# BatsResearch/menghini-neurips23-code

Measured on AMD Instinct MI355X. Metric: images/sec CLIP ViT-B/16 encode+prompt-step, higher is better.
Workload: dtype f16

## Files before the change

menghini-neurips23-code_amd/csrc/attention_split.hip:

```cpp
#include <math.h>

#include "common.h"

__device__ __forceinline__ int vt_index_fwd_s(int key, int d) { return vt_index(key, ((d >> 2) & 3) * 16 + (d >> 4) * 4 + (d & 3)); }

__device__ __forceinline__ void split8(const f32x4 a, const f32x4 b, half8& hi, half8& lo) {
    half4 h0, l0, h1, l1;
    split_f16x4(a, h0, l0);
    split_f16x4(b, h1, l1);
    hi = (half8){h0[0], h0[1], h0[2], h0[3], h1[0], h1[1], h1[2], h1[3]};
    lo = (half8){l0[0], l0[1], l0[2], l0[3], l1[0], l1[1], l1[2], l1[3]};
}

template <int KVC, bool CAUSAL, int NW>
__global__ __launch_bounds__(NW * 64) void attn_fwd_split_kernel(const float* __restrict__ qkv, half_t* __restrict__ out, int S, int H) {
    constexpr int SP = KVC * 32;
    constexpr float LOG2E = 1.4426950408889634f;
    constexpr float INV = 1.0f / (float)GRIP_SPLIT_LO_SCALE;
    extern __shared__ __attribute__((aligned(16))) char smem[];
    half_t* Kh = (half_t*)smem;
    half_t* Kl = Kh + SP * 64;
    half_t* Vh = Kl + SP * 64;
    half_t* Vl = Vh + SP * 64;

    const int tid = threadIdx.x, lane = tid & 63, wave = tid >> 6;
    const int D = H * 64;
    const int b = blockIdx.x / H, h = blockIdx.x - b * H;
    const size_t ld = (size_t)3 * D;
    const float* base = qkv + (size_t)b * S * ld + h * 64;
    const int li = lane & 15, lg = lane >> 4;
    const int n_qt = (S + 15) >> 4;

    for (int idx = tid; idx < SP * 8; idx += NW * 64) {
        const int row = idx >> 3, chunk = idx & 7;
        f32x4 a = {0.f, 0.f, 0.f, 0.f}, c = {0.f, 0.f, 0.f, 0.f};
        if (row < S) {
            const f32x4* p = (const f32x4*)(base + (size_t)row * ld + D + chunk * 8);
            a = p[0];
            c = p[1];
        }
        half8 hi, lo;
        split8(a, c, hi, lo);
        const int o = row * 64 + ((chunk ^ (row & 7)) * 8);
        *(half8*)(Kh + o) = hi;
        *(half8*)(Kl + o) = lo;
    }
    for (int idx = tid; idx < ((SP / 2 + 31) / 32) * 256; idx += NW * 64) {
        const int lane_rp = idx & 31, chunk = ((idx >> 5) & 1) + 2 * ((idx >> 6) & 3), rblk = idx >> 8;
        const int r0 = 2 * (rblk * 32 + lane_rp);
        if (r0 >= SP) continue;
        f32x4 z = {0.f, 0.f, 0.f, 0.f};
        f32x4 a0 = z, a1 = z, b0 = z, b1 = z;
        if (r0 < S) { const f32x4* p = (const f32x4*)(base + (size_t)r0 * ld + 2 * D + chunk * 8); a0 = p[0]; a1 = p[1]; }
        if (r0 + 1 < S) { const f32x4* p = (const f32x4*)(base + (size_t)(r0 + 1) * ld + 2 * D + chunk * 8); b0 = p[0]; b1 = p[1]; }
        half8 h0, l0, h1, l1;
        split8(a0, a1, h0, l0);
        split8(b0, b1, h1, l1);
#pragma unroll
        for (int j = 0; j < 8; ++j) {
            const int o = vt_index_fwd_s(r0, chunk * 8 + j);
            *(half2v*)(Vh + o) = (half2v){h0[j], h1[j]};
            *(half2v*)(Vl + o) = (half2v){l0[j], l1[j]};
        }
    }
    __syncthreads();

    for (int qt = wave; qt < n_qt; qt += NW) {
        asm volatile("" ::: "memory");
        const int qrow = qt * 16 + li;
        const int qr = qrow < S ? qrow : S - 1;
        half8 qh[2], ql[2];
#pragma unroll
        for (int kk = 0; kk < 2; ++kk) {
            const f32x4* p = (const f32x4*)(base + (size_t)qr * ld + (kk * 4 + lg) * 8);
            split8(p[0] * 0.125f, p[1] * 0.125f, qh[kk], ql[kk]);
        }
        f32x4 sc[2 * KVC];
        float m = -INFINITY;
#pragma unroll
        for (int t = 0; t < 2 * KVC; ++t) {
            f32x4 acc = {0.f, 0.f, 0.f, 0.f}, cor = {0.f, 0.f, 0.f, 0.f};
#pragma unroll
            for (int kk = 0; kk < 2; ++kk) {
                const int o = (t * 16 + li) * 64 + (((kk * 4 + lg) ^ (lane & 7)) * 8);
                const half8 kh = *(const half8*)(Kh + o), kl = *(const half8*)(Kl + o);
                acc = __builtin_amdgcn_mfma_f32_16x16x32_f16(kh, qh[kk], acc, 0, 0, 0);
                cor = __builtin_amdgcn_mfma_f32_16x16x32_f16(kl, qh[kk], cor, 0, 0, 0);
                cor = __builtin_amdgcn_mfma_f32_16x16x32_f16(kh, ql[kk], cor, 0, 0, 0);
            }
            acc += cor * INV;
            if (CAUSAL || t >= 2 * (KVC - 1)) {
#pragma unroll
                for (int r = 0; r < 4; ++r) {
                    const int kv = t * 16 + lg * 4 + r;
                    if (kv >= S || (CAUSAL && kv > qrow)) acc[r] = -INFINITY;
                }
            }
            m = fmaxf(fmaxf(fmaxf(m, acc[0]), fmaxf(acc[1], acc[2])), acc[3]);
            sc[t] = acc;
        }
        m = fmaxf(m, __shfl_xor(m, 16));
        m = fmaxf(m, __shfl_xor(m, 32));
        const float m2 = m * LOG2E;
#pragma unroll
        for (int t = 0; t < 2 * KVC; ++t)
#pragma unroll
            for (int r = 0; r < 4; ++r) sc[t][r] = __builtin_amdgcn_exp2f(__builtin_fmaf(sc[t][r], LOG2E, -m2));

        const half8 ones = {1, 1, 1, 1, 1, 1, 1, 1};
        f32x4 sum_h = {0.f, 0.f, 0.f, 0.f}, sum_l = {0.f, 0.f, 0.f, 0.f};
        f32x4 o[4], oc[4];
#pragma unroll
        for (int nf = 0; nf < 4; ++nf) { o[nf] = (f32x4){0.f, 0.f, 0.f, 0.f}; oc[nf] = (f32x4){0.f, 0.f, 0.f, 0.f}; }
#pragma unroll
        for (int c = 0; c < KVC; ++c) {
            half8 ph, pl;
            split8(sc[2 * c], sc[2 * c + 1], ph, pl);
#pragma unroll
            for (int nf = 0; nf < 4; ++nf) {
                const int vo = (c * 4 + nf) * 512 + (lg * 16 + (li ^ lg)) * 8;
                const half8 vh = *(const half8*)(Vh + vo), vl = *(const half8*)(Vl + vo);
                o[nf] = __builtin_amdgcn_mfma_f32_16x16x32_f16(vh, ph, o[nf], 0, 0, 0);
                oc[nf] = __builtin_amdgcn_mfma_f32_16x16x32_f16(vl, ph, oc[nf], 0, 0, 0);
                oc[nf] = __builtin_amdgcn_mfma_f32_16x16x32_f16(vh, pl, oc[nf], 0, 0, 0);
            }
            sum_h = __builtin_amdgcn_mfma_f32_16x16x32_f16(ones, ph, sum_h, 0, 0, 0);
            sum_l = __builtin_amdgcn_mfma_f32_16x16x32_f16(ones, pl, sum_l, 0, 0, 0);
        }
        if (qrow < S) {
            const float inv = 1.0f / (sum_h[0] + sum_l[0] * INV);
            half_t* orow = out + (size_t)((size_t)b * S + qrow) * 2 * D;
            const int col = h * 64 + lg * 16;
            half_t* op = orow + (col >> 5) * 64 + (col & 31);
            half8 hi0, lo0, hi1, lo1;
            split8((o[0] + oc[0] * INV) * inv, (o[1] + oc[1] * INV) * inv, hi0, lo0);
            split8((o[2] + oc[2] * INV) * inv, (o[3] + oc[3] * INV) * inv, hi1, lo1);
            *(half8*)op = hi0;
            *(half8*)(op + 8) = hi1;
            *(half8*)(op + 32) = lo0;
            *(half8*)(op + 40) = lo1;
        }
    }
}

bool attention_split_supported(int S) { return S >= 1 && S <= 320; }

int launch_attention_fwd_split(const float* qkv, void* out, int B, int S, int H, int causal, hipStream_t s) {
    GRIP_REQUIRE(attention_split_supported(S) && B >= 1 && H >= 1, "attention_split: bad shape B=%d S=%d H=%d (S <= 320)", B, S, H);
    const int kvc = (S + 31) / 32;
    const size_t lds = (size_t)4 * kvc * 32 * 64 * sizeof(half_t);
#define GRIP_ATT_CASE(K)                                                                                                                     \
    case K: {                                                                                                                                \
        static bool configured = false;                                                                                                      \
        if (!configured) {                                                                                                                   \
            GRIP_CHECK_HIP(hipFuncSetAttribute((const void*)attn_fwd_split_kernel<K, false, (K >= 4 ? 8 : 4)>, hipFuncAttributeMaxDynamicSharedMemorySize, (int)lds)); \
            GRIP_CHECK_HIP(hipFuncSetAttribute((const void*)attn_fwd_split_kernel<K, true, (K >= 4 ? 8 : 4)>, hipFuncAttributeMaxDynamicSharedMemorySize, (int)lds));  \
            configured = true;                                                                                                               \
        }                                                                                                                                    \
        if (causal) hipLaunchKernelGGL((attn_fwd_split_kernel<K, true, (K >= 4 ? 8 : 4)>), dim3(B * H), dim3((K >= 4 ? 8 : 4) * 64), lds, s, qkv, (half_t*)out, S, H); \
        else hipLaunchKernelGGL((attn_fwd_split_kernel<K, false, (K >= 4 ? 8 : 4)>), dim3(B * H), dim3((K >= 4 ? 8 : 4) * 64), lds, s, qkv, (half_t*)out, S, H);       \
    } break;
    switch (kvc) {
        GRIP_ATT_CASE(1) GRIP_ATT_CASE(2) GRIP_ATT_CASE(3) GRIP_ATT_CASE(4) GRIP_ATT_CASE(5)
        GRIP_ATT_CASE(6) GRIP_ATT_CASE(7) GRIP_ATT_CASE(8) GRIP_ATT_CASE(9) GRIP_ATT_CASE(10)
        default: GRIP_REQUIRE(false, "attention_split: S = %d out of range", S);
    }
#undef GRIP_ATT_CASE
    GRIP_CHECK_HIP(hipGetLastError());
    return GRIP_OK;
}
```

Before: 20760.

## Add persistent split-attention kernel overlapping next head's K/V loads with compute

```diff
diff --git a/menghini-neurips23-code_amd/csrc/attention_split.hip b/menghini-neurips23-code_amd/csrc/attention_split.hip
--- a/menghini-neurips23-code_amd/csrc/attention_split.hip
+++ b/menghini-neurips23-code_amd/csrc/attention_split.hip
@@ -12,11 +12,95 @@
     lo = (half8){l0[0], l0[1], l0[2], l0[3], l1[0], l1[1], l1[2], l1[3]};
 }
 
+template <int KVC, bool CAUSAL, class Store>
+__device__ __forceinline__ void attn_split_tile(const half_t* Kh, const half_t* Kl, const half_t* Vh, const half_t* Vl, const half8 (&qh)[2], const half8 (&ql)[2],
+                                                int qrow, int S, int lane, Store&& store) {
+    constexpr float LOG2E = 1.4426950408889634f;
+    constexpr float INV = 1.0f / (float)GRIP_SPLIT_LO_SCALE;
+    const int li = lane & 15, lg = lane >> 4;
+    f32x4 sc[2 * KVC];
+    float m = -INFINITY;
+    half8 kh[2][2], kl[2][2];
+    auto read_k = [&](int t) {
+#pragma unroll
+        for (int kk = 0; kk < 2; ++kk) {
+            const int o = (t * 16 + li) * 64 + (((kk * 4 + lg) ^ (lane & 7)) * 8);
+            kh[t & 1][kk] = *(const half8*)(Kh + o);
+            kl[t & 1][kk] = *(const half8*)(Kl + o);
+        }
+    };
+    read_k(0);
+#pragma unroll
+    for (int t = 0; t < 2 * KVC; ++t) {
+        if (t + 1 < 2 * KVC) read_k(t + 1);
+        f32x4 acc = {0.f, 0.f, 0.f, 0.f}, cor = {0.f, 0.f, 0.f, 0.f};
+#pragma unroll
+        for (int kk = 0; kk < 2; ++kk) {
+            acc = __builtin_amdgcn_mfma_f32_16x16x32_f16(kh[t & 1][kk], qh[kk], acc, 0, 0, 0);
+            cor = __builtin_amdgcn_mfma_f32_16x16x32_f16(kl[t & 1][kk], qh[kk], cor, 0, 0, 0);
+            cor = __builtin_amdgcn_mfma_f32_16x16x32_f16(kh[t & 1][kk], ql[kk], cor, 0, 0, 0);
+        }
+        acc += cor * INV;
+        if (CAUSAL || t >= 2 * (KVC - 1)) {
+#pragma unroll
+            for (int r = 0; r < 4; ++r) {
+                const int kv = t * 16 + lg * 4 + r;
+                if (kv >= S || (CAUSAL && kv > qrow)) acc[r] = -INFINITY;
+            }
+        }
+        m = fmaxf(fmaxf(fmaxf(m, acc[0]), fmaxf(acc[1], acc[2])), acc[3]);
+        sc[t] = acc;
+    }
+    m = fmaxf(m, __shfl_xor(m, 16));
+    m = fmaxf(m, __shfl_xor(m, 32));
+    const float m2 = m * LOG2E;
+#pragma unroll
+    for (int t = 0; t < 2 * KVC; ++t)
+#pragma unroll
+        for (int r = 0; r < 4; ++r) sc[t][r] = __builtin_amdgcn_exp2f(__builtin_fmaf(sc[t][r], LOG2E, -m2));
+
+    const half8 ones = {1, 1, 1, 1, 1, 1, 1, 1};
+    f32x4 sum_h = {0.f, 0.f, 0.f, 0.f}, sum_l = {0.f, 0.f, 0.f, 0.f};
+    f32x4 o[4], oc[4];
+#pragma unroll
+    for (int nf = 0; nf < 4; ++nf) { o[nf] = (f32x4){0.f, 0.f, 0.f, 0.f}; oc[nf] = (f32x4){0.f, 0.f, 0.f, 0.f}; }
+    half8 vh[2], vl[2];
+    auto read_v = [&](int st) {
+        const int vo = st * 512 + (lg * 16 + (li ^ lg)) * 8;
+        vh[st & 1] = *(const half8*)(Vh + vo);
+        vl[st & 1] = *(const half8*)(Vl + vo);
+    };
+    read_v(0);
+#pragma unroll
+    for (int c = 0; c < KVC; ++c) {
+        half8 ph, pl;
+        split8(sc[2 * c], sc[2 * c + 1], ph, pl);
+#pragma unroll
+        for (int nf = 0; nf < 4; ++nf) {
+            const int st = c * 4 + nf;
+            if (st + 1 < 4 * KVC) read_v(st + 1);
+            o[nf] = __builtin_amdgcn_mfma_f32_16x16x32_f16(vh[st & 1], ph, o[nf], 0, 0, 0);
+            oc[nf] = __builtin_amdgcn_mfma_f32_16x16x32_f16(vl[st & 1], ph, oc[nf], 0, 0, 0);
+            oc[nf] = __builtin_amdgcn_mfma_f32_16x16x32_f16(vh[st & 1], pl, oc[nf], 0, 0, 0);
+        }
+        sum_h = __builtin_amdgcn_mfma_f32_16x16x32_f16(ones, ph, sum_h, 0, 0, 0);
+        sum_l = __builtin_amdgcn_mfma_f32_16x16x32_f16(ones, pl, sum_l, 0, 0, 0);
+    }
+    const float inv = 1.0f / (sum_h[0] + sum_l[0] * INV);
+    half8 hi0, lo0, hi1, lo1;
+    split8((o[0] + oc[0] * INV) * inv, (o[1] + oc[1] * INV) * inv, hi0, lo0);
+    split8((o[2] + oc[2] * INV) * inv, (o[3] + oc[3] * INV) * inv, hi1, lo1);
+    store(hi0, hi1, lo0, lo1);
+}
+
+__device__ __forceinline__ int split_out_col(int h, int lane) {
+    const int col = h * 64 + (lane >> 4) * 16;
+    return (col >> 5) * 64 + (col & 31);
+}
+
 template <int KVC, bool CAUSAL, int NW>
 __global__ __launch_bounds__(NW * 64) void attn_fwd_split_kernel(const float* __restrict__ qkv, half_t* __restrict__ out, int S, int H) {
     constexpr int SP = KVC * 32;
-    constexpr float LOG2E = 1.4426950408889634f;
-    constexpr float INV = 1.0f / (float)GRIP_SPLIT_LO_SCALE;
     extern __shared__ __attribute__((aligned(16))) char smem[];
     half_t* Kh = (half_t*)smem;
     half_t* Kl = Kh + SP * 64;
@@ -65,6 +149,7 @@
     }
     __syncthreads();
 
+    half_t* orow = out + (size_t)b * S * 2 * D + split_out_col(h, lane);
     for (int qt = wave; qt < n_qt; qt += NW) {
         asm volatile("" ::: "memory");
         const int qrow = qt * 16 + li;
@@ -75,79 +160,225 @@
             const f32x4* p = (const f32x4*)(base + (size_t)qr * ld + (kk * 4 + lg) * 8);
             split8(p[0] * 0.125f, p[1] * 0.125f, qh[kk], ql[kk]);
         }
-        f32x4 sc[2 * KVC];
-        float m = -INFINITY;
-#pragma unroll
-        for (int t = 0; t < 2 * KVC; ++t) {
-            f32x4 acc = {0.f, 0.f, 0.f, 0.f}, cor = {0.f, 0.f, 0.f, 0.f};
-#pragma unroll
-            for (int kk = 0; kk < 2; ++kk) {
-                const int o = (t * 16 + li) * 64 + (((kk * 4 + lg) ^ (lane & 7)) * 8);
-                const half8 kh = *(const half8*)(Kh + o), kl = *(const half8*)(Kl + o);
-                acc = __builtin_amdgcn_mfma_f32_16x16x32_f16(kh, qh[kk], acc, 0, 0, 0);
-                cor = __builtin_amdgcn_mfma_f32_16x16x32_f16(kl, qh[kk], cor, 0, 0, 0);
-                cor = __builtin_amdgcn_mfma_f32_16x16x32_f16(kh, ql[kk], cor, 0, 0, 0);
+        attn_split_tile<KVC, CAUSAL>(Kh, Kl, Vh, Vl, qh, ql, qrow, S, lane, [&](half8 hi0, half8 hi1, half8 lo0, half8 lo1) {
+            if (qrow < S) {
+                half_t* op = orow + (size_t)qrow * 2 * D;
+                *(half8*)op = hi0;
+                *(half8*)(op + 8) = hi1;
+                *(half8*)(op + 32) = lo0;
+                *(half8*)(op + 40) = lo1;
             }
-            acc += cor * INV;
-            if (CAUSAL || t >= 2 * (KVC - 1)) {
-#pragma unroll
-                for (int r = 0; r < 4; ++r) {
-                    const int kv = t * 16 + lg * 4 + r;
-                    if (kv >= S || (CAUSAL && kv > qrow)) acc[r] = -INFINITY;
+        });
+    }
+}
+
+template <int KVC>
+__global__ __launch_bounds__(512) void attn_fwd_split_persistent_kernel(const float* __restrict__ qkv, half_t* __restrict__ out, int S, int H, int n_items) {
+    constexpr int NW = 8;
+    constexpr int SP = KVC * 32;
+    constexpr int NK = SP * 16 / (NW * 64);
+    constexpr int V_UNITS = ((SP / 2 + 31) / 32) * 256;
+    constexpr int NV = (V_UNITS + NW * 64 - 1) / (NW * 64);
+    static_assert(2 * KVC > NW && 2 * KVC <= 2 * NW, "one or two query tiles per wave");
+    extern __shared__ __attribute__((aligned(16))) char smem[];
+    half_t* Kh = (half_t*)smem;
+    half_t* Kl = Kh + SP * 64;
+    half_t* Vh = Kl + SP * 64;
+    half_t* Vl = Vh + SP * 64;
+
+    const int tid = threadIdx.x;
+    const int wave = __builtin_amdgcn_readfirstlane(tid >> 6);
+    const int D = H * 64;
+    const size_t ld = (size_t)3 * D;
+    const int n_qt = (S + 15) >> 4;
+
+    f32x4 kr[NK], vr[NV][4];
+    f32x4 qr[2][2];
+    half8 qh[2], ql[2];
+    const unsigned ldb = (unsigned)ld * 4;
+    const unsigned odb = (unsigned)D * 4;
+    auto fresh_tid = [&]() {
+        int t = tid;
+        asm volatile("" : "+v"(t));
+        return t;
+    };
+    auto in_rsrc = [&](int item) {
+        const int b = __builtin_amdgcn_readfirstlane(item / H), h = item - b * H;
+        return __builtin_amdgcn_make_buffer_rsrc((void*)(qkv + (size_t)b * S * ld + h * 64), 0, (int)((unsigned)(S - 1) * ldb + (unsigned)(2 * D + 64) * 4), 0x00020000);
+    };
+    auto out_rsrc = [&](int item) {
+        const int b = __builtin_amdgcn_readfirstlane(item / H);
+        return __builtin_amdgcn_make_buffer_rsrc((void*)(out + (size_t)b * S * 2 * D), 0, (int)((unsigned)S * odb), 0x00020000);
+    };
+    auto ldg = [&](__amdgpu_buffer_rsrc_t rs, unsigned off) { return __builtin_bit_cast(f32x4, __builtin_amdgcn_raw_buffer_load_b128(rs, (int)off, 0, 0)); };
+    auto load_k = [&](__amdgpu_buffer_rsrc_t rs) {
+        const int t = fresh_tid();
+        const unsigned ko = (unsigned)(t >> 4) * ldb + (unsigned)(D + (t & 15) * 4) * 4;
+#pragma unroll
+        for (int n = 0; n < NK; ++n) kr[n] = ldg(rs, ko + n * 32 * ldb);
+    };
+    auto load_v = [&](__amdgpu_buffer_rsrc_t rs) {
+        const int t = fresh_tid();
+        const int v_r0 = 2 * ((t >> 8) * 32 + (t & 31)), v_chunk = ((t >> 5) & 1) + 2 * ((t >> 6) & 3);
+        const unsigned vo = (unsigned)v_r0 * ldb + (unsigned)(2 * D + v_chunk * 8) * 4;
+#pragma unroll
+        for (int n = 0; n < NV; ++n) {
+            vr[n][0] = ldg(rs, vo + n * 128 * ldb);
+            vr[n][1] = ldg(rs, vo + n * 128 * ldb + 16);
+            vr[n][2] = ldg(rs, vo + (n * 128 + 1) * ldb);
+            vr[n][3] = ldg(rs, vo + (n * 128 + 1) * ldb + 16);
+        }
+    };
+    auto load_q = [&](__amdgpu_buffer_rsrc_t rs, int qt) {
+        const int t = fresh_tid();
+        const int qrow = qt * 16 + (t & 15);
+        const unsigned q_off = (unsigned)(qrow < S ? qrow : S - 1) * ldb + (unsigned)((t >> 4) & 3) * 32;
+#pragma unroll
+        for (int kk = 0; kk < 2; ++kk) {
+            qr[kk][0] = ldg(rs, q_off + kk * 128);
+            qr[kk][1] = ldg(rs, q_off + kk * 128 + 16);
+        }
+    };
+    auto split_q = [&]() {
+#pragma unroll
+        for (int kk = 0; kk < 2; ++kk) split8(qr[kk][0] * 0.125f, qr[kk][1] * 0.125f, qh[kk], ql[kk]);
+    };
+    auto stage_kv = [&]() {
+        const int t = fresh_tid();
+        const int k_r0 = t >> 4, k_q = t & 15;
+        half_t* kp = Kh + k_r0 * 64 + (((k_q >> 1) ^ (k_r0 & 7)) * 8) + (k_q & 1) * 4;
+#pragma unroll
+        for (int n = 0; n < NK; ++n) {
+            half4 hi, lo;
+            split_f16x4(kr[n], hi, lo);
+            *(half4*)(kp + n * 2048) = hi;
+            *(half4*)(kp + n * 2048 + SP * 64) = lo;
+        }
+        const int v_r0 = 2 * ((t >> 8) * 32 + (t & 31)), v_chunk = ((t >> 5) & 1) + 2 * ((t >> 6) & 3);
+        const int v_lg = (v_r0 >> 2) & 3;
+        const int v_lds = vt_index_fwd_s(v_r0, v_chunk * 8) ^ (v_lg * 8);
+        int v_st[4];
+#pragma unroll
+        for (int jj = 0; jj < 4; ++jj) {
+            v_st[jj] = 2 * SP * 64 + v_lds + ((jj ^ v_lg) * 8);
+            asm volatile("" : "+v"(v_st[jj]));
+        }
+        half8 vh[NV][2], vl[NV][2];
+#pragma unroll
+        for (int n = 0; n < NV; ++n) {
+            split8(vr[n][0], vr[n][1], vh[n][0], vl[n][0]);
+            split8(vr[n][2], vr[n][3], vh[n][1], vl[n][1]);
+        }
+#pragma unroll
+        for (int n = 0; n < NV; ++n) {
+            if (v_r0 + n * 128 < SP) {
+#pragma unroll
+                for (int j = 0; j < 8; ++j) {
+                    half_t* o = Kh + v_st[j & 3] + (n * 8192 + (j >> 2) * 512);
+                    *(half2v*)o = (half2v){vh[n][0][j], vh[n][1][j]};
+                    *(half2v*)(o + SP * 64) = (half2v){vl[n][0][j], vl[n][1][j]};
                 }
             }
-            m = fmaxf(fmaxf(fmaxf(m, acc[0]), fmaxf(acc[1], acc[2])), acc[3]);
-            sc[t] = acc;
-        }
-        m = fmaxf(m, __shfl_xor(m, 16));
-        m = fmaxf(m, __shfl_xor(m, 32));
-        const float m2 = m * LOG2E;
-#pragma unroll
-        for (int t = 0; t < 2 * KVC; ++t)
-#pragma unroll
-            for (int r = 0; r < 4; ++r) sc[t][r] = __builtin_amdgcn_exp2f(__builtin_fmaf(sc[t][r], LOG2E, -m2));
-
-        const half8 ones = {1, 1, 1, 1, 1, 1, 1, 1};
-        f32x4 sum_h = {0.f, 0.f, 0.f, 0.f}, sum_l = {0.f, 0.f, 0.f, 0.f};
-        f32x4 o[4], oc[4];
-#pragma unroll
-        for (int nf = 0; nf < 4; ++nf) { o[nf] = (f32x4){0.f, 0.f, 0.f, 0.f}; oc[nf] = (f32x4){0.f, 0.f, 0.f, 0.f}; }
-#pragma unroll
-        for (int c = 0; c < KVC; ++c) {
-            half8 ph, pl;
-            split8(sc[2 * c], sc[2 * c + 1], ph, pl);
-#pragma unroll
-            for (int nf = 0; nf < 4; ++nf) {
-                const int vo = (c * 4 + nf) * 512 + (lg * 16 + (li ^ lg)) * 8;
-                const half8 vh = *(const half8*)(Vh + vo), vl = *(const half8*)(Vl + vo);
-                o[nf] = __builtin_amdgcn_mfma_f32_16x16x32_f16(vh, ph, o[nf], 0, 0, 0);
-                oc[nf] = __builtin_amdgcn_mfma_f32_16x16x32_f16(vl, ph, oc[nf], 0, 0, 0);
-                oc[nf] = __builtin_amdgcn_mfma_f32_16x16x32_f16(vh, pl, oc[nf], 0, 0, 0);
-            }
-            sum_h = __builtin_amdgcn_mfma_f32_16x16x32_f16(ones, ph, sum_h, 0, 0, 0);
-            sum_l = __builtin_amdgcn_mfma_f32_16x16x32_f16(ones, pl, sum_l, 0, 0, 0);
-        }
-        if (qrow < S) {
-            const float inv = 1.0f / (sum_h[0] + sum_l[0] * INV);
-            half_t* orow = out + (size_t)((size_t)b * S + qrow) * 2 * D;
-            const int col = h * 64 + lg * 16;
-            half_t* op = orow + (col >> 5) * 64 + (col & 31);
-            half8 hi0, lo0, hi1, lo1;
-            split8((o[0] + oc[0] * INV) * inv, (o[1] + oc[1] * INV) * inv, hi0, lo0);
-            split8((o[2] + oc[2] * INV) * inv, (o[3] + oc[3] * INV) * inv, hi1, lo1);
-            *(half8*)op = hi0;
-            *(half8*)(op + 8) = hi1;
-            *(half8*)(op + 32) = lo0;
-            *(half8*)(op + 40) = lo1;
-        }
+        }
+    };
+    auto tile = [&](int item, int qt) {
+        const int ln = fresh_tid() & 63;
+        const int h = item - __builtin_amdgcn_readfirstlane(item / H) * H;
+        const __amdgpu_buffer_rsrc_t ors = out_rsrc(item);
+        const int qrow = qt * 16 + (ln & 15);
+        const unsigned oo = qrow < S ? (unsigned)qrow * odb + (unsigned)split_out_col(h, ln) * 2 : 0x40000000u;
+        asm volatile("" ::: "memory");
+        attn_split_tile<KVC, false>(Kh, Kl, Vh, Vl, qh, ql, qrow, S, ln, [&](half8 hi0, half8 hi1, half8 lo0, half8 lo1) {
+            typedef unsigned u32x4 __attribute__((ext_vector_type(4)));
+            __builtin_amdgcn_raw_buffer_store_b128(__builtin_bit_cast(u32x4, hi0), ors, (int)oo, 0, 0);
+            __builtin_amdgcn_raw_buffer_store_b128(__builtin_bit_cast(u32x4, hi1), ors, (int)(oo + 16), 0, 0);
+            __builtin_amdgcn_raw_buffer_store_b128(__builtin_bit_cast(u32x4, lo0), ors, (int)(oo + 64), 0, 0);
+            __builtin_amdgcn_raw_buffer_store_b128(__builtin_bit_cast(u32x4, lo1), ors, (int)(oo + 80), 0, 0);
+        });
+    };
+    auto plane_barrier = [&]() {
+        asm volatile("s_waitcnt lgkmcnt(0)" ::: "memory");
+        __builtin_amdgcn_s_barrier();
+        asm volatile("" ::: "memory");
+    };
+
+    int item = blockIdx.x;
+    if (item >= n_items) return;
+    const bool second = wave + NW < n_qt;
+    {
+        const __amdgpu_buffer_rsrc_t rs = in_rsrc(item);
+        load_k(rs);
+        load_v(rs);
+        load_q(rs, wave);
+        stage_kv();
+        split_q();
+    }
+    for (;;) {
+        plane_barrier();
+        const int next = item + gridDim.x;
+        if (next >= n_items) break;
+        const __amdgpu_buffer_rsrc_t nrs = in_rsrc(next);
+        load_k(nrs);
+        if (second) {
+            load_q(in_rsrc(item), wave + NW);
+            tile(item, wave);
+            load_v(nrs);
+            split_q();
+            load_q(nrs, wave);
+            tile(item, wave + NW);
+            plane_barrier();
+            stage_kv();
+            split_q();
+        } else {
+            tile(item, wave);
+            load_v(nrs);
+            load_q(nrs, wave);
+            plane_barrier();
+            stage_kv();
+            split_q();
+        }
+        item = next;
+    }
+    if (second) load_q(in_rsrc(item), wave + NW);
+    tile(item, wave);
+    if (second) {
+        split_q();
+        tile(item, wave + NW);
     }
 }
 
 bool attention_split_supported(int S) { return S >= 1 && S <= 320; }
+
+template <int KVC>
+static int launch_split_persistent(const float* qkv, half_t* out, int B, int S, int H, hipStream_t s) {
+    constexpr size_t lds = (size_t)4 * KVC * 32 * 64 * sizeof(half_t);
+    static int resident = 0, per_cu_s = 0;
+    if (!resident) {
+        GRIP_CHECK_HIP(hipFuncSetAttribute((const void*)attn_fwd_split_persistent_kernel<KVC>, hipFuncAttributeMaxDynamicSharedMemorySize, (int)lds));
+        int dev = 0, n_cu = 0, per_cu = 0;
+        GRIP_CHECK_HIP(hipGetDevice(&dev));
+        GRIP_CHECK_HIP(hipDeviceGetAttribute(&n_cu, hipDeviceAttributeMultiprocessorCount, dev));
+        GRIP_CHECK_HIP(hipOccupancyMaxActiveBlocksPerMultiprocessor(&per_cu, attn_fwd_split_persistent_kernel<KVC>, 512, lds));
+        GRIP_REQUIRE(per_cu >= 1, "attention_split: persistent kernel does not fit a CU (KVC %d)", KVC);
+        resident = n_cu * per_cu;
+        per_cu_s = per_cu;
+    }
+    const int n_items = B * H;
+    const int width = (grip_cu_budget() > 0 && grip_cu_budget() * per_cu_s < resident) ? grip_cu_budget() * per_cu_s : resident;
+    const int grid = n_items < width ? n_items : width;
+    hipLaunchKernelGGL((attn_fwd_split_persistent_kernel<KVC>), dim3(grid), dim3(512), lds, s, qkv, out, S, H, n_items);
+    GRIP_CHECK_HIP(hipGetLastError());
+    return GRIP_OK;
+}
 
 int launch_attention_fwd_split(const float* qkv, void* out, int B, int S, int H, int causal, hipStream_t s) {
     GRIP_REQUIRE(attention_split_supported(S) && B >= 1 && H >= 1, "attention_split: bad shape B=%d S=%d H=%d (S <= 320)", B, S, H);
     const int kvc = (S + 31) / 32;
+    if (!causal) {
+        if (kvc == 5) return launch_split_persistent<5>(qkv, (half_t*)out, B, S, H, s);
+        if (kvc == 6) return launch_split_persistent<6>(qkv, (half_t*)out, B, S, H, s);
+        if (kvc == 7) return launch_split_persistent<7>(qkv, (half_t*)out, B, S, H, s);
+    }
     const size_t lds = (size_t)4 * kvc * 32 * 64 * sizeof(half_t);
 #define GRIP_ATT_CASE(K)                                                                                                                     \
     case K: {                                                                                                                                \
```

Result: no change. 20870 (median of 6 runs) (+0.6%).
